# xyloid/a_dive_into_ray_tracing

Hardware: AMD Instinct MI355X
Metric: Msamples/sec (pixels x spp) on RTIOW final scene (higher is better)
Workload: dtype f32

## Files before the change

### a_dive_into_ray_tracing_amd/csrc/rtmi_device.hip

```cpp
#include <hip/hip_runtime.h>
#include <hipcub/hipcub.hpp>

#include <algorithm>
#include <cmath>
#include <cstdint>
#include <cstdlib>
#include <cstdio>
#include <cstring>
#include <memory>
#include <mutex>
#include <string>
#include <vector>

#include "rtmi_internal.h"
#include "rtmi_path.h"


namespace rtmi {

struct RenderArgs {
  Cam<float> cam;
  int32_t n, npairs, W, H, spp, max_depth;
  uint64_t seed;
  int32_t row0, row_step, nrows_valid;
  int32_t tiles_x, n_items;
  int32_t tiles, spp1, chunk1, nch1, chunk2, nch2;
  int32_t block_flush;
  int32_t block_owns_tile;
  int32_t acc_off;
  int32_t s_base;
  uint64_t out_elems;
  Accel acc;
  const int32_t *tile_order;
  unsigned *tile_cost;
};

#ifndef RTMI_WAVES_PER_BLOCK
#define RTMI_WAVES_PER_BLOCK 4
#endif
constexpr int kWavesPerBlock = RTMI_WAVES_PER_BLOCK;
#ifndef RTMI_WAVES_PER_EU
#define RTMI_WAVES_PER_EU 1
#endif
#ifndef RTMI_TRACE
#define RTMI_TRACE 0
#endif
#if RTMI_TRACE
constexpr unsigned kTraceCap = 1u << 18;
__device__ unsigned long long g_trace[kTraceCap * 4];
// ... 121 lines not shown
  atomicAdd(&segments[2], (unsigned long long)cnt.bvh_stats[3]);
  atomicAdd(&segments[4], (unsigned long long)cnt.bvh_stats[4]);
#else
  (void)cnt, (void)lane, (void)segments;
#endif
}

constexpr bool acc_grid(int A) { return A >= 2; }
constexpr bool acc_flat(int A) { return A == 3 || A == 5; }
constexpr bool acc_gmem(int A) { return A >= 4; }

template <int ACC, bool FIRST = false>
__device__ __forceinline__ bool path_segment(const SceneView<float> &sc, const SpherePair *__restrict__ pairs,
                                             const RenderArgs &a, V3<float> &o, V3<float> &d, V3<float> &T,
                                             int &depth, Xoro &rng, V3<float> &col, SegCounters &cnt,
                                             unsigned long long *segments) {
  (void)cnt, (void)segments;
  float t;
#if RTMI_TRACE
  const unsigned long long cyc0 = __builtin_amdgcn_s_memtime();
#endif
  int k;
  uint32_t key = 0u;
  if constexpr (ACC == 1) {
    k = hit_world_bvh<kBigGroup>(a.acc, o, d, t
#if RTMI_STATS
                                  , cnt.bvh_stats
#endif
    );
  } else if constexpr (ACC >= 2) {
    k = hit_world_grid<kBigGroup, acc_flat(ACC), acc_gmem(ACC)>(a.acc, o, d, t, key
#if RTMI_STATS
                                   , cnt.bvh_stats
#endif
#if RTMI_TRACE_PHASES
                                   , cnt.pc
#endif
                                   );
  } else {
    k = hit_world_packed<kPairGroup>(pairs, a.npairs, o, d, t
#if RTMI_STATS
                                     , cnt.stats
#endif
    );
  }
#if RTMI_TRACE
  if constexpr (!(RTMI_TRACE_PHASES && acc_grid(ACC))) cnt.cyc_hit += __builtin_amdgcn_s_memtime() - cyc0;
#endif
#if RTMI_CHECK
  if (k >= a.n) atomicAdd(&segments[7], 1ull << 32);
#endif
  const bool miss = k < 0 || (RTMI_CHECK && k >= a.n);
  const int kk = miss ? 0 : k;
// ... 73 lines not shown
      const int i2 = it - a.tiles * a.nch1;
      tl = i2 / a.nch2;
      sb = a.spp1 + (i2 - tl * a.nch2) * a.chunk2;
      n = max(0, min(a.chunk2, a.spp - sb));
    }
  };
  int tile, s0, ns;
  item_range(has_item ? item : 0, tile, s0, ns);
  if (!has_item) ns = 0;
  if (a.tile_order) tile = a.tile_order[tile];
  const int ty = tile / a.tiles_x, tx = tile - ty * a.tiles_x;
  const int x0 = tx * TW, y0 = ty * TH;
  const int vw = min(TW, a.W - x0), vh = min(TH, a.nrows_valid - y0);
  const int nv = vw * vh;
  const int nq = nv * ns;

  unsigned nseg = 0;
  RTMI_TRACE_BEGIN
  SegCounters cnt{};
#if RTMI_TRACE_PHASES
  unsigned long long cyc_iter = 0, cyc_regen = 0, cyc_ramp = 0;
#endif

  const SceneView<float> sc{geom, sh0, sh1, a.n};

  V3<float> o, d, T;
  int pxd = 0;
  bool active = true;
  Xoro rng;

// ... 44 lines not shown
      unsigned below = 0;
      asm volatile("" : "+s"(below));
      return int(__builtin_amdgcn_mbcnt_hi(~0u, __builtin_amdgcn_mbcnt_lo(~0u, below)));
    };
    const int q = pbase + lane_now();
    const int nvalid = min(64, nq - pbase);
    if constexpr (BATCH) {
#if RTMI_TRACE_PHASES
      const unsigned long long cyc_r = __builtin_amdgcn_s_memtime();
#endif
      bool survives = false;
      if (q < nq) {
        camera_ray(q, po, pd, prng);
        V3<float> unused_T = mk(1.f, 1.f, 1.f), col = mk(0.f, 0.f, 0.f);
        int hit = 0;
        survives = !path_segment<ACC, true>(sc, pairs, a, po, pd, unused_T, hit, prng, col, cnt, segments);
        const int px = job_pixel(pbase + lane_now());
        ptag = px | (hit << 6);
        if (!survives) {
          atomicAdd(&acc[px], (unsigned long long)to_fixed(col.x));
          atomicAdd(&acc[64 + px], (unsigned long long)to_fixed(col.y));
          atomicAdd(&acc[128 + px], (unsigned long long)to_fixed(col.z));
        }
      }
      nseg = unsigned(__builtin_amdgcn_readfirstlane(int(nseg + unsigned(nvalid))));
      const unsigned long long m = __ballot(survives);
      plive = __popcll(m);
      const int rank = __builtin_amdgcn_mbcnt_hi(unsigned(m >> 32), __builtin_amdgcn_mbcnt_lo(unsigned(m), 0u));
      const int dst4 = (survives ? rank : plive + lane_now() - rank) << 2;
      po = mk(push(dst4, po.x), push(dst4, po.y), push(dst4, po.z));
      pd = mk(push(dst4, pd.x), push(dst4, pd.y), push(dst4, pd.z));
// ... 709 lines not shown
  BvhNode *nodes = nullptr;
  int32_t nnodes = 0;
  bool bvh_global = false;
  bool force_bvh_global = std::getenv("RTMI_BVH_GLOBAL") && std::atoi(std::getenv("RTMI_BVH_GLOBAL")) != 0;
  float4 *bvh_sph = nullptr;
  int32_t *bvh_idx = nullptr;
  int32_t nbvh_sph = 0;
  float4 *grid_sph = nullptr;
  uint32_t *grid_cells = nullptr;
  uint32_t *grid_refs = nullptr;
  GridDesc grid{};
  int32_t ngrid_sph = 0;
  bool grid_ok = false;
  bool grid_global = false;
  char *grid_gmem = nullptr;
  bool force_grid_global = std::getenv("RTMI_GRID_GLOBAL") && std::atoi(std::getenv("RTMI_GRID_GLOBAL")) != 0;
  int32_t ordering = RT_ORDER_COST;
  bool block_flush = !(std::getenv("RTMI_BLOCK_FLUSH") && std::getenv("RTMI_BLOCK_FLUSH")[0] == '0');
  bool block_owns = !(std::getenv("RTMI_BLOCK_OWNS") && std::getenv("RTMI_BLOCK_OWNS")[0] == '0');
  int32_t last_sched[8] = {0, 0, 0, 0, 0, 0, 0, 0};
  unsigned *cost_prev = nullptr, *cost_cur = nullptr, *cost_sorted = nullptr;
  int32_t *order = nullptr, *iota = nullptr;
  size_t cost_cap = 0;
  void *sort_tmp = nullptr;
  size_t sort_tmp_bytes = 0;
  bool cost_valid = false;
  int64_t cost_key[6] = {0, 0, 0, 0, 0, 0};
  hipStream_t last_stream = nullptr;
  hipEvent_t last_done = nullptr;
  int32_t tile_w = 0;
// ... 96 lines not shown
    ctx->cu_count = prop.multiProcessorCount;
  }
  *out = ctx.release();
  return RT_OK;
}

RTMI_EXPORT int rt_ctx_destroy(rt_ctx *ctx) {
  if (!ctx) return RT_OK;
  DeviceGuard guard(ctx->device);
  (void)hipStreamSynchronize(ctx->stream);
  for (void *p : {(void *)ctx->geom, (void *)ctx->sh0, (void *)ctx->sh1, (void *)ctx->geom64, (void *)ctx->sh064,
                  (void *)ctx->sh164, (void *)ctx->accum, (void *)ctx->scratch, (void *)ctx->segments, (void *)ctx->pairs, (void *)ctx->counter, (void *)ctx->pass_accum,
                  (void *)ctx->big_pairs, (void *)ctx->big_idx, (void *)ctx->nodes, (void *)ctx->bvh_sph, (void *)ctx->bvh_idx,
                  (void *)ctx->cost_prev, (void *)ctx->cost_cur, (void *)ctx->cost_sorted, (void *)ctx->order,
                  (void *)ctx->iota, ctx->sort_tmp, (void *)ctx->grid_sph, (void *)ctx->grid_cells, (void *)ctx->grid_refs,
                  (void *)ctx->grid_gmem})
    if (p) (void)hipFree(p);
  (void)hipStreamDestroy(ctx->stream);
  if (ctx->last_done) (void)hipEventDestroy(ctx->last_done);
  delete ctx;
  return RT_OK;
}

namespace {
constexpr size_t kBvhLdsMax = 64 * 1024;

uint16_t half_bits(_Float16 h) { return __builtin_bit_cast(uint16_t, h); }
uint16_t half_down(double v) {
  _Float16 h = _Float16(v);
  while (double(h) > v) {
    uint16_t b = half_bits(h);
// ... 80 lines not shown
      build(ids + best_mid, cnt - best_mid);
      nd.link = int32_t(nodes.size());
    }
    nodes[me] = nd;
  }
};
}

namespace {
struct GridBuild {
  GridDesc desc{};
  std::vector<float4> sph;
  std::vector<uint32_t> cells;
  std::vector<uint32_t> refs;
  bool fits_lds = true;
};
bool build_grid(const BvhBuilder &b, const std::vector<int32_t> &small, int32_t n, int32_t nbig_slots,
                GridBuild &out) {
  if (n > 65535) return false;
  const char *env = std::getenv("RTMI_GRID_CELLS");
  const double per_sphere = env && std::atof(env) > 0 ? std::atof(env) : 0.3;
  double lo[3] = {INFINITY, INFINITY, INFINITY}, hi[3] = {-INFINITY, -INFINITY, -INFINITY};
  for (int32_t k : small) {
    const double *c = b.cr + 4 * k, R = std::fabs(c[3]) + b.margin(k);
    for (int a = 0; a < 3; ++a) {
      lo[a] = std::min(lo[a], c[a] - R);
      hi[a] = std::max(hi[a], c[a] + R);
    }
  }
  double e[3], vol = 1;
// ... 36 lines not shown
      for (int y = c0[1]; y <= c1[1]; ++y)
        for (int x = c0[0]; x <= c1[0]; ++x)
          lists[size_t(x + out.desc.n[0] * (y + out.desc.n[1] * z))].push_back(uint16_t(k));
  }
  out.sph.assign(b.g.begin(), b.g.begin() + n);
  out.cells.resize(size_t(total) + 1);
  for (int64_t cidx = 0; cidx < total; ++cidx) {
    out.cells[size_t(cidx)] = uint32_t(out.refs.size());
    for (uint16_t k : lists[size_t(cidx)]) out.refs.push_back(uint32_t(k) * 16u);
  }
  out.cells[size_t(total)] = uint32_t(out.refs.size());
  out.desc.nrefs = int32_t(out.refs.size());
  out.desc.cells_off = 16u * uint32_t(nbig_slots + out.desc.nrefs);
  out.desc.idx_off = out.desc.cells_off + 4u * uint32_t(out.desc.ncells + 1);
  const char *lim_env = std::getenv("RTMI_GRID_LDS_MAX");
  const size_t lds_max = lim_env && std::atoll(lim_env) > 0 ? size_t(std::atoll(lim_env)) : 160 * 1024 / 8 - 3 * 64 * 8 - 256;
  out.fits_lds = grid_lds_bytes(nbig_slots, out.desc.ncells, out.desc.nrefs) <= lds_max;
  return true;
}
}

RTMI_EXPORT int rt_ctx_set_ordering(rt_ctx *ctx, int32_t ordering) {
  if (!ctx) return set_error(RT_EINVAL, "null ctx");
  if (ordering != RT_ORDER_NONE && ordering != RT_ORDER_COST) return set_error(RT_EINVAL, "unknown ordering %d", ordering);
  ctx->ordering = ordering;
  ctx->cost_valid = false;
  return RT_OK;
}

RTMI_EXPORT int rt_ctx_set_accel(rt_ctx *ctx, int32_t accel) {
  if (!ctx) return set_error(RT_EINVAL, "null ctx");
  if (accel != RT_ACCEL_NONE && accel != RT_ACCEL_BVH && accel != RT_ACCEL_GRID)
    return set_error(RT_EINVAL, "unknown accel %d", accel);
// ... 115 lines not shown
    ctx->grid_ok = false;
    GridBuild gb;
    if (!small.empty() && build_grid(b, small, n, nb_pad, gb)) {
      if ((rc = dev_alloc(&ctx->grid_sph, gb.sph.size())) || (rc = dev_alloc(&ctx->grid_cells, gb.cells.size())) ||
          (rc = dev_alloc(&ctx->grid_refs, std::max<size_t>(gb.refs.size(), 1))))
        return rc;
      HIP_TRY(hipMemcpy(ctx->grid_sph, gb.sph.data(), gb.sph.size() * sizeof(float4), hipMemcpyHostToDevice));
      HIP_TRY(hipMemcpy(ctx->grid_cells, gb.cells.data(), gb.cells.size() * sizeof(uint32_t), hipMemcpyHostToDevice));
      if (!gb.refs.empty())
        HIP_TRY(hipMemcpy(ctx->grid_refs, gb.refs.data(), gb.refs.size() * sizeof(uint32_t), hipMemcpyHostToDevice));
      ctx->grid = gb.desc;
      ctx->grid.cells = ctx->grid_cells;
      ctx->grid.refs = ctx->grid_refs;
      ctx->ngrid_sph = int32_t(gb.sph.size());
      ctx->grid_global = ctx->force_grid_global || !gb.fits_lds;
      if (ctx->grid_global) {
        const int32_t nbs = nb_pad, nrec = nbs + gb.desc.nrefs;
        std::vector<char> img(grid_lds_bytes(nbs, gb.desc.ncells, gb.desc.nrefs), 0);
        float4 *rec = reinterpret_cast<float4 *>(img.data());
        uint32_t *cst = reinterpret_cast<uint32_t *>(img.data() + gb.desc.cells_off);
        uint16_t *ix = reinterpret_cast<uint16_t *>(img.data() + gb.desc.idx_off);
        for (int32_t i = 0; i < nrec; ++i) {
          const int32_t k = i < nbs ? bidx[size_t(i)] : int32_t(gb.refs[size_t(i - nbs)] >> 4);
          rec[i] = k < 0 ? make_float4(0.f, 0.f, 0.f, 0.f) : gb.sph[size_t(k)];
          ix[i] = uint16_t(k < 0 ? 0 : k);
        }
        for (int32_t i = 0; i <= gb.desc.ncells; ++i) cst[i] = 16u * (uint32_t(nbs) + gb.cells[size_t(i)]);
        if ((rc = dev_alloc(&ctx->grid_gmem, img.size()))) return rc;
        HIP_TRY(hipMemcpy(ctx->grid_gmem, img.data(), img.size(), hipMemcpyHostToDevice));
      }
// ... 11 lines not shown
  if (n_refs) *n_refs = ctx->grid.nrefs;
  if (lds_bytes) *lds_bytes = int32_t(grid_lds_bytes(2 * ctx->nbig_pairs, ctx->grid.ncells, ctx->grid.nrefs));
  return RT_OK;
}

RTMI_EXPORT int rt_debug_grid_strides(const int32_t *n3, uint32_t *strides2) {
  if (!n3 || !strides2) return set_error(RT_EINVAL, "rt_debug_grid_strides: bad argument");
  GridDesc d{};
  for (int a = 0; a < 3; ++a) d.n[a] = n3[a];
  if (!grid_strides(d)) return set_error(RT_EINVAL, "grid of %d x %d x %d cells: over the walk's 24-bit bound", n3[0], n3[1], n3[2]);
  strides2[0] = d.row_bytes;
  strides2[1] = d.layer_bytes;
  return RT_OK;
}

RTMI_EXPORT int rt_debug_grid_layout(const rt_scene *scene, int32_t *dims3, uint32_t *strides2, float *box6) {
  if (!scene || scene->n <= 0 || !scene->center_radius || !dims3 || !strides2)
    return set_error(RT_EINVAL, "rt_debug_grid_layout: bad argument");
  const int n = scene->n;
  std::vector<float4> g(n, make_float4(0.f, 0.f, 0.f, 0.f));
  std::vector<double> rad(n);
  for (int k = 0; k < n; k++) rad[k] = std::fabs(scene->center_radius[4 * k + 3]);
  std::vector<double> sorted_r = rad;
  std::nth_element(sorted_r.begin(), sorted_r.begin() + n / 2, sorted_r.end());
  const double med = sorted_r[n / 2];
  std::vector<int32_t> big, small;
  double scale = 0;
  for (int k = 0; k < n; k++) {
    (rad[k] > RTMI_BIG_FACTOR * med ? big : small).push_back(k);
    for (int a = 0; a < 3; ++a) scale = std::max(scale, std::fabs(scene->center_radius[4 * k + a]) + rad[k]);
  }
  BvhBuilder b{scene->center_radius, g, 1e-6 * scale, {}, {}, {}};
  const int nb_pad = big.empty() ? 0 : (int(big.size()) + 2 * kBigGroup - 1) / (2 * kBigGroup) * (2 * kBigGroup);
  GridBuild gb;
  if (small.empty() || !build_grid(b, small, n, nb_pad, gb)) return set_error(RT_EUNSUPPORTED, "no grid for this scene");
  for (int a = 0; a < 3; ++a) dims3[a] = gb.desc.n[a];
  strides2[0] = gb.desc.row_bytes;
  strides2[1] = gb.desc.layer_bytes;
  if (box6)
    for (int a = 0; a < 3; ++a) {
      box6[a] = gb.desc.g0[a];
      box6[3 + a] = gb.desc.h[a];
    }
  return RT_OK;
}

RTMI_EXPORT int rt_ctx_set_schedule(rt_ctx *ctx, int32_t chunk, int32_t tail_spp, int32_t tail_chunk) {
  if (!ctx) return set_error(RT_EINVAL, "null ctx");
  if (chunk < 0 || tail_chunk < 0) return set_error(RT_EINVAL, "chunk sizes must be >= 0");
  ctx->chunk = chunk;
// ... 12 lines not shown
RTMI_EXPORT int rt_ctx_set_kernel(rt_ctx *ctx, int32_t kind) {
  if (!ctx) return set_error(RT_EINVAL, "null ctx");
  if (kind != RT_KERNEL_GRID && kind != RT_KERNEL_PERSISTENT && kind != RT_KERNEL_AUTO && kind != RT_KERNEL_QUEUE &&
      kind != RT_KERNEL_RESIDENT)
    return set_error(RT_EINVAL, "unknown kernel kind");
  ctx->kernel = kind;
  return RT_OK;
}

static int auto_tile_w(int32_t W, int32_t rows) {
  auto idle = [&](int64_t tw) {
    const int64_t th = 64 / tw;
    return ((W + tw - 1) / tw) * tw * ((rows + th - 1) / th) * th - int64_t(W) * rows;
  };
  return idle(16) < idle(8) ? 16 : 8;
}

RTMI_EXPORT int rt_ctx_set_tuning(rt_ctx *ctx, int32_t tile_w, int32_t chunk) {
  if (!ctx) return set_error(RT_EINVAL, "null ctx");
  if (tile_w != 0 && tile_w != 8 && tile_w != 16 && tile_w != 32 && tile_w != 64)
    return set_error(RT_EINVAL, "tile_w must be 0 (automatic), 8, 16, 32 or 64");
  if (chunk < 0) return set_error(RT_EINVAL, "chunk must be >= 0");
  ctx->tile_w = tile_w;
  ctx->chunk = chunk;
  return RT_OK;
}

namespace {

size_t accel_lds_bytes(const Accel &acc, int kind) {
// ... 5 lines not shown

Accel accel_of(const rt_ctx *ctx, int kind) {
  Accel a{ctx->big_pairs, ctx->big_idx, ctx->nbig_pairs, 0, nullptr, nullptr, nullptr, 0, GridDesc{}};
  if (kind == 1) {
    a.nnodes = ctx->nnodes;
    a.nodes = ctx->nodes;
    a.sph = ctx->bvh_sph;
    a.sph_idx = ctx->bvh_idx;
    a.nsph = ctx->nbvh_sph;
    a.bvh_global = ctx->bvh_global;
  } else if (kind >= 2) {
    a.sph = ctx->grid_sph;
    a.nsph = ctx->ngrid_sph;
    a.grid = ctx->grid;
    a.grid_gmem = ctx->grid_global ? ctx->grid_gmem : nullptr;
  }
  return a;
}

template <int TW>
void launch_persistent(bool chunked, dim3 grid, hipStream_t st, const rt_ctx *ctx, const RenderArgs &a,
                       unsigned long long *accum, float *out) {
  if (chunked)
    hipLaunchKernelGGL((render_persistent<TW, true>), grid, dim3(64 * kWavesPerBlock), 0, st, ctx->geom, ctx->sh0,
                       ctx->sh1, ctx->pairs, a, accum, out, ctx->segments, ctx->counter);
  else
    hipLaunchKernelGGL((render_persistent<TW, false>), grid, dim3(64 * kWavesPerBlock), 0, st, ctx->geom, ctx->sh0,
                       ctx->sh1, ctx->pairs, a, accum, out, ctx->segments, ctx->counter);
}

template <int TW, int ACC>
void launch_tw(bool chunked, dim3 grid, hipStream_t st, const rt_ctx *ctx, const RenderArgs &a,
               unsigned long long *accum, float *out) {
  RenderArgs b = a;
  b.acc_off = int32_t((accel_lds_bytes(a.acc, ACC) + 15) / 16 * 16);
  const size_t lds = size_t(b.acc_off) + size_t(chunked && a.block_flush ? 1 : GridShape<ACC != 0>::waves) * 3 * 64 * 8;
  if (chunked)
    hipLaunchKernelGGL((render_kernel<TW, true, ACC>), grid, dim3(64 * GridShape<ACC != 0>::waves), lds, st, ctx->geom,
                       ctx->sh0, ctx->sh1, ctx->pairs, b, accum, out, ctx->segments);
  else
    hipLaunchKernelGGL((render_kernel<TW, false, ACC>), grid, dim3(64 * GridShape<ACC != 0>::waves), lds, st, ctx->geom,
                       ctx->sh0, ctx->sh1, ctx->pairs, b, accum, out, ctx->segments);
}

#if RTMI_EXPERIMENTAL
int res_resident_blocks(rt_ctx *ctx, size_t dyn) {
  if (ctx->res_blocks <= 0 || ctx->res_lds != dyn) {
    int per_cu = 0;
    if (hipOccupancyMaxActiveBlocksPerMultiprocessor(&per_cu, (const void *)render_resident<8, 3>, 64 * kResWaves,
                                                     dyn) != hipSuccess)
      per_cu = 0;
// ... 112 lines not shown
  a.npairs = ctx->npairs;
  a.W = W; a.H = H; a.spp = spp; a.max_depth = max_depth; a.seed = seed;
  a.row0 = row0; a.row_step = row_step; a.nrows_valid = nvalid;
  a.tiles_x = tiles_x; a.n_items = int32_t(items);
  a.tiles = int32_t(tiles); a.spp1 = spp1; a.chunk1 = chunk1; a.nch1 = nch1; a.chunk2 = chunk2; a.nch2 = nch2;
  a.block_flush = !persistent && !resident && nch1 % grid_wpb == 0 && nch2 % grid_wpb == 0 && ctx->block_flush;
  a.block_owns_tile = a.block_flush && !pass_accum && nch1 == grid_wpb && nch2 == 0 && ctx->block_owns;
  if (resident) a.block_owns_tile = !pass_accum && nch1 == 1 && nch2 == 0 && ctx->block_owns;
  const bool chunked = pass_accum || nch1 + nch2 > 1;
  if (!ctx->probing) {
    const int32_t sched[8] = {TW, chunk1, nch1, nch2, a.block_flush + a.block_owns_tile, persistent ? 0 : 1,
                              resident ? 3 : (persistent ? 1 : 0), acc_kind == 3 ? 2 : (acc_kind == 5 ? 4 : acc_kind)};
    std::copy(sched, sched + 8, ctx->last_sched);
  }
  a.s_base = s_base;
  a.out_elems = uint64_t(nvalid) * uint64_t(W) * 3;
  const size_t n_valid_out = size_t(nvalid) * W * 3;
  if (chunked && !pass_accum && !a.block_owns_tile) {
    if (ctx->accum_cap < n_valid_out) {
      int rc = dev_alloc(&ctx->accum, n_valid_out);
      if (rc) { ctx->accum_cap = 0; return rc; }
      ctx->accum_cap = n_valid_out;
    }
  }
  unsigned long long *const accum = pass_accum ? pass_accum : ctx->accum;
  if (chunked && !a.block_owns_tile && (!accum || (pass_accum ? ctx->pass_cap : ctx->accum_cap) < n_valid_out))
    return set_error(RT_EHIP, "internal: accumulator not allocated for %zu elements", n_valid_out);
  if ((!chunked || a.block_owns_tile) && !strip) return set_error(RT_EHIP, "internal: no output strip");
  if (int64_t(tiles_y) * TH < nvalid || int64_t(tiles_x) * TW < W || nch1 * int64_t(chunk1) < spp1 ||
      nch2 * int64_t(chunk2) < spp - spp1)
// ... 483 lines not shown
```

### a_dive_into_ray_tracing_amd/csrc/rtmi_path.h

```cpp
#pragma once

#include <hip/hip_runtime.h>

#include <cmath>
#include <cstdint>
#include <type_traits>

#include "../../include/rtmi.h"

#ifndef RTMI_STATS
#define RTMI_STATS 0
#endif

namespace rtmi {


constexpr int kGeomPad = 16;

template <class R> struct V3 { R x, y, z; };
template <class R> __host__ __device__ __forceinline__ V3<R> mk(R x, R y, R z) { return V3<R>{x, y, z}; }

template <bool F> __device__ __forceinline__ float madd(float a, float b, float c) {
  if constexpr (F) return __builtin_fmaf(a, b, c);
  else return a * b + c;
// ... 337 lines not shown
  return true;
}

struct Accel {
  const SpherePair *big;
  const int32_t *big_idx;
  int32_t nbig_pairs;
  int32_t nnodes;
  const BvhNode *nodes;
  const float4 *sph;
  const int32_t *sph_idx;
  int32_t nsph;
  GridDesc grid;
  int32_t bvh_global;
  const char *grid_gmem;
};

__device__ __forceinline__ int32_t big_index(const Accel &a, int slot) {
  typedef const __attribute__((address_space(4))) int32_t *cidx_t;
  return ((cidx_t)(size_t)a.big_idx)[slot];
}

extern __shared__ float4 rtmi_bvh_lds[];
__host__ __device__ constexpr size_t bvh_lds_bytes(int32_t nnodes, int32_t nsph) {
  return size_t(nnodes + nsph) * 16 + size_t(nsph) * 2;
}

__device__ __forceinline__ void stage_bvh(const Accel &g) {
  if (!g.bvh_global) {
    const float4 *nodes = reinterpret_cast<const float4 *>(g.nodes);
    for (int i = threadIdx.x; i < g.nnodes; i += blockDim.x) rtmi_bvh_lds[i] = nodes[i];
// ... 164 lines not shown
      auto res = [&](int slot, float hb, float disc) {
        if constexpr (KEYS)
          resolve_root(int32_t((GMEM ? 0u : lds_address(rtmi_bvh_lds)) + 16u * uint32_t(slot)), hb, disc, inv_a, t_max,
                       best);
        else
          resolve_root(big_index(acc_s, slot), hb, disc, inv_a, t_max, best);
      };
      if (m & 1u) res(2 * q, hb0.x, d0.x);
      if (m & 2u) res(2 * q + 1, hb0.y, d0.y);
      if (m & 4u) res(2 * q + 2, hb1.x, d1.x);
      if (m & 8u) res(2 * q + 3, hb1.y, d1.y);
    }
  }
}

template <int GP, bool FLAT_Y = false, bool GMEM = false>
__device__ __forceinline__ int32_t hit_world_grid(const Accel &acc_s, V3<float> o, V3<float> d, float &t_hit,
                                                  uint32_t &hit_key
#if RTMI_STATS
                                                  , unsigned *gstats
#endif
#if RTMI_TRACE_PHASES
                                                  , PhaseClock &pc
#endif
                                                  ) {
#if RTMI_TRACE_PHASES
  const unsigned long long tp0 = __builtin_amdgcn_s_memtime();
#endif
  RTMI_RAY_TERMS(o, d)
  const char *const gm = GMEM ? acc_s.grid_gmem : nullptr;
  const uint32_t base = GMEM ? 0u : lds_address(rtmi_bvh_lds), idx_base = base + acc_s.grid.idx_off;
  auto rd_u32 = [&](uint32_t addr) {
    if constexpr (GMEM) return *reinterpret_cast<const uint32_t *>(gm + addr);
    else return lds_u32(addr);
  };
  auto rd_u16 = [&](uint32_t addr) {
    if constexpr (GMEM) return uint32_t(*reinterpret_cast<const uint16_t *>(gm + addr));
    else return lds_u16(addr);
  };
  auto rd_sphere = [&](uint32_t addr) {
    if constexpr (GMEM) return *reinterpret_cast<const float4 *>(gm + addr);
    else return lds_sphere(addr);
  };
  float t_max = INFINITY;
  int32_t best_a = -1;
  hit_big<GP, true, GMEM>(acc_s, d, K, a, aL, mx, my, mz, inv_a, t_max, best_a
#if RTMI_STATS
              , gstats
#endif
              );
#if RTMI_TRACE_PHASES
  const unsigned long long tp1 = __builtin_amdgcn_s_memtime();
  pc.c[0] += tp1 - tp0;
  unsigned long long tp2 = tp1;
#endif
  const GridDesc &G = rtmi_grid_desc;
  const float ix = safe_inv<FLAT_Y>(d.x), iy = safe_inv<FLAT_Y>(d.y), iz = safe_inv<FLAT_Y>(d.z);
  const float ox = -o.x * ix, oy = -o.y * iy, oz = -o.z * iz;
  const float bx0 = __builtin_fmaf(G.g0[0], ix, ox), bx1 = __builtin_fmaf(G.g1[0], ix, ox);
  const float by0 = __builtin_fmaf(G.g0[1], iy, oy), by1 = __builtin_fmaf(G.g1[1], iy, oy);
  const float bz0 = __builtin_fmaf(G.g0[2], iz, oz), bz1 = __builtin_fmaf(G.g1[2], iz, oz);
  const float tnear = __builtin_fmaxf(__builtin_fmaxf(__builtin_fminf(bx0, bx1), __builtin_fminf(by0, by1)),
                                      __builtin_fmaxf(__builtin_fminf(bz0, bz1), 0.0f));
  const float tfar = __builtin_fminf(__builtin_fminf(__builtin_fmaxf(bx0, bx1), __builtin_fmaxf(by0, by1)),
                                     __builtin_fminf(__builtin_fmaxf(bz0, bz1), t_max));
  if (tnear <= tfar) {
    const uint32_t cells = base + G.cells_off;
    auto cell_of = [&](float p, int ax) {
      return __builtin_amdgcn_fmed3f(__builtin_floorf((p - G.g0[ax]) * G.inv_h[ax]), 0.0f, G.nm1[ax]);
    };
    const float fx = cell_of(__builtin_fmaf(tnear, d.x, o.x), 0);
    const float fy = FLAT_Y ? 0.0f : cell_of(__builtin_fmaf(tnear, d.y, o.y), 1);
    const float fz = cell_of(__builtin_fmaf(tnear, d.z, o.z), 2);
    const int cx = int(fx), cy = int(fy), cz = int(fz);
    float t0x, t0y, t0z, dtx, dty, dtz, kmx, kmy, kmz;
    auto axis = [&](float inv, float oo, float cf, int ax, float &t0, float &dt, float &kmax) {
      const bool pos = inv >= 0.0f;
      t0 = __builtin_fmaf(__builtin_fmaf(pos ? cf + 1.0f : cf, G.h[ax], G.g0[ax]), inv, oo);
      dt = __builtin_fabsf(G.h[ax] * inv);
      kmax = pos ? G.nm1[ax] - cf : cf;
    };
    axis(ix, ox, fx, 0, t0x, dtx, kmx);
    if constexpr (FLAT_Y) {
      t0y = __builtin_fmaf(__builtin_fmaf(iy >= 0.0f ? 1.0f : 0.0f, G.h[1], G.g0[1]), iy, oy);
      dty = kmy = 0.0f;
    } else {
      axis(iy, oy, fy, 1, t0y, dty, kmy);
    }
    axis(iz, oz, fz, 2, t0z, dtz, kmz);
    float kx = 0.0f, ky = 0.0f, kz = 0.0f, tnx = t0x, tny = t0y, tnz = t0z;
    uint32_t cell = cells + 4u * uint32_t(cx) + __umul24(uint32_t(cz), G.layer_bytes);
    if constexpr (!FLAT_Y) cell += __umul24(uint32_t(cy), G.row_bytes);
    const int dcx = ix >= 0.0f ? 4 : -4;
    const int dcy = FLAT_Y ? 0 : (iy >= 0.0f ? int(G.row_bytes) : -int(G.row_bytes));
    const int dcz = iz >= 0.0f ? int(G.layer_bytes) : -int(G.layer_bytes);
#if RTMI_TRACE_PHASES
    tp2 = __builtin_amdgcn_s_memtime();
#endif
    for (;;) {
#if RTMI_STATS
      gstats[0] += 1;
      if (__lane_id() == __builtin_ctzll(__ballot(1))) gstats[2] += 1;
#endif
      const uint32_t re = rd_u32(cell + 4u);
      constexpr uint32_t kNoKey = 0xFFFFFFFFu;
      uint32_t kaddr = kNoKey;
      float khb = 0.0f, kdisc = 0.0f;
      for (uint32_t r = rd_u32(cell); r < re; r += 16u) {
#if RTMI_STATS
        gstats[1] += 1;
        if (__lane_id() == __builtin_ctzll(__ballot(1))) gstats[3] += 1;
#endif
        float hb, disc;
        sphere_test(rd_sphere(r), d, K, a, aL, mx, my, mz, hb, disc);
        if (!(disc < 0.0f)) {
          if (kaddr != kNoKey) {
#if RTMI_STATS
            if (__lane_id() == __builtin_ctzll(__ballot(1))) gstats[4] += 1;
#endif
            resolve_key<GMEM>(kaddr, khb, kdisc, inv_a, t_max, best_a, idx_base, gm);
          }
          kaddr = r;
          khb = hb;
          kdisc = disc;
        }
      }
      if (kaddr != kNoKey) {
#if RTMI_STATS
        if (__lane_id() == __builtin_ctzll(__ballot(1))) gstats[4] += 1;
#endif
        resolve_key<GMEM>(kaddr, khb, kdisc, inv_a, t_max, best_a, idx_base, gm);
      }
      const float texit = __builtin_fminf(tnx, __builtin_fminf(tny, tnz));
      if constexpr (FLAT_Y) {
        const bool sx = (tnx <= tny) & (tnx <= tnz);
        const bool sy = !sx & (tny <= tnz);
        const bool leave = !(texit < t_max) | sy | ((sx ? kx : kz) >= (sx ? kmx : kmz));
        if (leave) break;
        kx = sx ? kx + 1.0f : kx;
        kz = sx ? kz : kz + 1.0f;
        tnx = sx ? __builtin_fmaf(kx, dtx, t0x) : tnx;
        tnz = sx ? tnz : __builtin_fmaf(kz, dtz, t0z);
        cell += sx ? dcx : dcz;
        continue;
      }
      if (!(texit < t_max)) break;
      if (tnx <= tny && tnx <= tnz) {
        if (kx >= kmx) break;
        kx += 1.0f;
        tnx = __builtin_fmaf(kx, dtx, t0x);
        cell += dcx;
      } else if (tny <= tnz) {
        if (FLAT_Y || ky >= kmy) break;
        ky += 1.0f;
        tny = __builtin_fmaf(ky, dty, t0y);
        cell += dcy;
      } else {
        if (kz >= kmz) break;
        kz += 1.0f;
        tnz = __builtin_fmaf(kz, dtz, t0z);
        cell += dcz;
      }
    }
  }
#if RTMI_TRACE_PHASES
  {
    const unsigned long long tp3 = __builtin_amdgcn_s_memtime();
    pc.c[1] += tp2 - tp1;
    pc.c[2] += tp3 - tp2;
  }
#endif
  t_hit = t_max;
  hit_key = best_a < 0 ? base : uint32_t(best_a);
  const int32_t k = int32_t(rd_u16(idx_base + ((hit_key - base) >> 3)));
  return best_a < 0 ? -1 : k;
}
// ... 191 lines not shown
```

Measured before the change: 27710.

## Add per-tile camera-ray candidate sphere lists to skip grid traversal

Before tracing a tile, each wave builds a conservative list of small spheres that any primary ray from that tile's pixel cone could hit, and stores their LDS record keys in a per-wave LDS region. First-bounce grid hits then test only those candidates instead of walking the grid cells. The list is used only when it fits the cap and the tile has enough samples. This adds a per-tile culling pass over all small spheres, extra LDS, and a smaller grid LDS budget. For tiles with many candidates it falls back to normal traversal.

```diff
diff --git a/a_dive_into_ray_tracing_amd/csrc/rtmi_device.hip b/a_dive_into_ray_tracing_amd/csrc/rtmi_device.hip
--- a/a_dive_into_ray_tracing_amd/csrc/rtmi_device.hip
+++ b/a_dive_into_ray_tracing_amd/csrc/rtmi_device.hip
@@ -33,6 +33,7 @@
   Accel acc;
   const int32_t *tile_order;
   unsigned *tile_cost;
+  int32_t tile_list_max;
 };
 
 #ifndef RTMI_WAVES_PER_BLOCK
@@ -184,8 +185,8 @@
 __device__ __forceinline__ bool path_segment(const SceneView<float> &sc, const SpherePair *__restrict__ pairs,
                                              const RenderArgs &a, V3<float> &o, V3<float> &d, V3<float> &T,
                                              int &depth, Xoro &rng, V3<float> &col, SegCounters &cnt,
-                                             unsigned long long *segments) {
-  (void)cnt, (void)segments;
+                                             unsigned long long *segments, int32_t tile_list = -1) {
+  (void)cnt, (void)segments, (void)tile_list;
   float t;
 #if RTMI_TRACE
   const unsigned long long cyc0 = __builtin_amdgcn_s_memtime();
@@ -199,14 +200,14 @@
 #endif
     );
   } else if constexpr (ACC >= 2) {
-    k = hit_world_grid<kBigGroup, acc_flat(ACC), acc_gmem(ACC)>(a.acc, o, d, t, key
+    k = hit_world_grid<kBigGroup, acc_flat(ACC), acc_gmem(ACC), FIRST && !acc_gmem(ACC)>(a.acc, o, d, t, key
 #if RTMI_STATS
                                    , cnt.bvh_stats
 #endif
 #if RTMI_TRACE_PHASES
                                    , cnt.pc
 #endif
-                                   );
+                                   , tile_list);
   } else {
     k = hit_world_packed<kPairGroup>(pairs, a.npairs, o, d, t
 #if RTMI_STATS
@@ -310,6 +311,35 @@
   const int vw = min(TW, a.W - x0), vh = min(TH, a.nrows_valid - y0);
   const int nv = vw * vh;
   const int nq = nv * ns;
+
+  int32_t tile_list = -1;
+  if constexpr (ACC == 2 || ACC == 3) {
+    uint16_t *const tl = reinterpret_cast<uint16_t *>(acc_lds + (acc_shared ? 1 : WPB) * 3 * 64) + wave * kTileListCap;
+    const int cap = min(a.tile_list_max, kTileListCap);
+    if (cap > 0 && ns >= kTileListMinSpp && a.acc.ntile > 0) {
+      const TileBundle tb = tile_bundle(a.cam, a.W, a.H, x0, vw, a.row0 + y0 * a.row_step,
+                                        a.row0 + (y0 + vh - 1) * a.row_step);
+      const uint32_t *const keys = reinterpret_cast<const uint32_t *>(a.acc.tile_sph + a.acc.ntile);
+      const int ln = int(__builtin_amdgcn_mbcnt_hi(~0u, __builtin_amdgcn_mbcnt_lo(~0u, 0u)));
+      int n = 0;
+      for (int i0 = 0; i0 < a.acc.ntile && n <= cap; i0 += 64) {
+        const int i = i0 + ln;
+        bool pass = false;
+        uint32_t key = 0u;
+        if (i < a.acc.ntile) {
+          const float4 s = a.acc.tile_sph[i];
+          key = keys[i];
+          pass = tile_may_hit(tb, s.x, s.y, s.z, s.w);
+        }
+        const unsigned long long m = __ballot(pass);
+        const int slot = n + int(__builtin_amdgcn_mbcnt_hi(unsigned(m >> 32), __builtin_amdgcn_mbcnt_lo(unsigned(m), 0u)));
+        if (pass && slot < cap) tl[slot] = uint16_t(key);
+        n = __builtin_amdgcn_readfirstlane(n + __popcll(m));
+      }
+      __builtin_amdgcn_fence(__ATOMIC_RELEASE, "wavefront");
+      if (n <= cap) tile_list = __builtin_amdgcn_readfirstlane(int(lds_address(tl) << 6) | n);
+    }
+  }
 
   unsigned nseg = 0;
   RTMI_TRACE_BEGIN
@@ -384,7 +414,7 @@
         camera_ray(q, po, pd, prng);
         V3<float> unused_T = mk(1.f, 1.f, 1.f), col = mk(0.f, 0.f, 0.f);
         int hit = 0;
-        survives = !path_segment<ACC, true>(sc, pairs, a, po, pd, unused_T, hit, prng, col, cnt, segments);
+        survives = !path_segment<ACC, true>(sc, pairs, a, po, pd, unused_T, hit, prng, col, cnt, segments, tile_list);
         const int px = job_pixel(pbase + lane_now());
         ptag = px | (hit << 6);
         if (!survives) {
@@ -1124,6 +1154,11 @@
   bool grid_ok = false;
   bool grid_global = false;
   char *grid_gmem = nullptr;
+  float4 *tile_sph = nullptr;
+  int32_t ntile = 0;
+  int32_t tile_list_max = std::getenv("RTMI_TILE_LIST_MAX")
+                              ? std::max(0, std::min(kTileListCap, std::atoi(std::getenv("RTMI_TILE_LIST_MAX"))))
+                              : kTileListCap;
   bool force_grid_global = std::getenv("RTMI_GRID_GLOBAL") && std::atoi(std::getenv("RTMI_GRID_GLOBAL")) != 0;
   int32_t ordering = RT_ORDER_COST;
   bool block_flush = !(std::getenv("RTMI_BLOCK_FLUSH") && std::getenv("RTMI_BLOCK_FLUSH")[0] == '0');
@@ -1250,7 +1285,7 @@
                   (void *)ctx->big_pairs, (void *)ctx->big_idx, (void *)ctx->nodes, (void *)ctx->bvh_sph, (void *)ctx->bvh_idx,
                   (void *)ctx->cost_prev, (void *)ctx->cost_cur, (void *)ctx->cost_sorted, (void *)ctx->order,
                   (void *)ctx->iota, ctx->sort_tmp, (void *)ctx->grid_sph, (void *)ctx->grid_cells, (void *)ctx->grid_refs,
-                  (void *)ctx->grid_gmem})
+                  (void *)ctx->grid_gmem, (void *)ctx->tile_sph})
     if (p) (void)hipFree(p);
   (void)hipStreamDestroy(ctx->stream);
   if (ctx->last_done) (void)hipEventDestroy(ctx->last_done);
@@ -1361,6 +1396,8 @@
   std::vector<uint32_t> cells;
   std::vector<uint32_t> refs;
   bool fits_lds = true;
+  std::vector<float4> tile_sph;
+  std::vector<uint32_t> tile_keys;
 };
 bool build_grid(const BvhBuilder &b, const std::vector<int32_t> &small, int32_t n, int32_t nbig_slots,
                 GridBuild &out) {
@@ -1427,9 +1464,32 @@
   out.desc.cells_off = 16u * uint32_t(nbig_slots + out.desc.nrefs);
   out.desc.idx_off = out.desc.cells_off + 4u * uint32_t(out.desc.ncells + 1);
   const char *lim_env = std::getenv("RTMI_GRID_LDS_MAX");
-  const size_t lds_max = lim_env && std::atoll(lim_env) > 0 ? size_t(std::atoll(lim_env)) : 160 * 1024 / 8 - 3 * 64 * 8 - 256;
+  const size_t lds_max = lim_env && std::atoll(lim_env) > 0
+                             ? size_t(std::atoll(lim_env))
+                             : 160 * 1024 / 8 - 3 * 64 * 8 - 256 - GridShape<true>::waves * 2 * kTileListCap;
   out.fits_lds = grid_lds_bytes(nbig_slots, out.desc.ncells, out.desc.nrefs) <= lds_max;
+  std::vector<uint32_t> first(size_t(n), UINT32_MAX);
+  for (size_t p = out.refs.size(); p-- > 0;) first[out.refs[p] >> 4] = uint32_t(nbig_slots) + uint32_t(p);
+  if (size_t(nbig_slots) + out.refs.size() <= 65536) {
+    for (int32_t k : small) {
+      const double *c = b.cr + 4 * k, R = std::fabs(c[3]) + b.margin(k);
+      float rg = float(R);
+      if (double(rg) < R) rg = std::nextafter(rg, INFINITY);
+      out.tile_sph.push_back(make_float4(float(c[0]), float(c[1]), float(c[2]), rg));
+      out.tile_keys.push_back(first[size_t(k)]);
+    }
+  }
   return true;
+}
+
+void tile_extent(int32_t W, int32_t row0, int32_t row_step, int32_t nvalid, int32_t tw, int32_t tile, int32_t &x0,
+                 int32_t &vw, int32_t &j_lo, int32_t &j_hi) {
+  const int32_t th = 64 / tw, tiles_x = (W + tw - 1) / tw, ty = tile / tiles_x, tx = tile - ty * tiles_x;
+  const int32_t y0 = ty * th, vh = std::min(th, nvalid - y0);
+  x0 = tx * tw;
+  vw = std::min(tw, W - x0);
+  j_lo = row0 + y0 * row_step;
+  j_hi = row0 + (y0 + vh - 1) * row_step;
 }
 }
 
@@ -1575,6 +1635,16 @@
       ctx->grid.refs = ctx->grid_refs;
       ctx->ngrid_sph = int32_t(gb.sph.size());
       ctx->grid_global = ctx->force_grid_global || !gb.fits_lds;
+      ctx->ntile = 0;
+      if (!ctx->grid_global && !gb.tile_sph.empty()) {
+        const size_t ns = gb.tile_sph.size();
+        std::vector<float4> tab(ns + (ns + 3) / 4);
+        std::copy(gb.tile_sph.begin(), gb.tile_sph.end(), tab.begin());
+        std::memcpy(tab.data() + ns, gb.tile_keys.data(), ns * sizeof(uint32_t));
+        if ((rc = dev_alloc(&ctx->tile_sph, tab.size()))) return rc;
+        HIP_TRY(hipMemcpy(ctx->tile_sph, tab.data(), tab.size() * sizeof(float4), hipMemcpyHostToDevice));
+        ctx->ntile = int32_t(ns);
+      }
       if (ctx->grid_global) {
         const int32_t nbs = nb_pad, nrec = nbs + gb.desc.nrefs;
         std::vector<char> img(grid_lds_bytes(nbs, gb.desc.ncells, gb.desc.nrefs), 0);
@@ -1616,9 +1686,8 @@
   return RT_OK;
 }
 
-RTMI_EXPORT int rt_debug_grid_layout(const rt_scene *scene, int32_t *dims3, uint32_t *strides2, float *box6) {
-  if (!scene || scene->n <= 0 || !scene->center_radius || !dims3 || !strides2)
-    return set_error(RT_EINVAL, "rt_debug_grid_layout: bad argument");
+namespace {
+bool host_grid(const rt_scene *scene, GridBuild &gb, int32_t &nbs) {
   const int n = scene->n;
   std::vector<float4> g(n, make_float4(0.f, 0.f, 0.f, 0.f));
   std::vector<double> rad(n);
@@ -1633,9 +1702,17 @@
     for (int a = 0; a < 3; ++a) scale = std::max(scale, std::fabs(scene->center_radius[4 * k + a]) + rad[k]);
   }
   BvhBuilder b{scene->center_radius, g, 1e-6 * scale, {}, {}, {}};
-  const int nb_pad = big.empty() ? 0 : (int(big.size()) + 2 * kBigGroup - 1) / (2 * kBigGroup) * (2 * kBigGroup);
+  nbs = big.empty() ? 0 : (int(big.size()) + 2 * kBigGroup - 1) / (2 * kBigGroup) * (2 * kBigGroup);
+  return !small.empty() && build_grid(b, small, n, nbs, gb);
+}
+}
+
+RTMI_EXPORT int rt_debug_grid_layout(const rt_scene *scene, int32_t *dims3, uint32_t *strides2, float *box6) {
+  if (!scene || scene->n <= 0 || !scene->center_radius || !dims3 || !strides2)
+    return set_error(RT_EINVAL, "rt_debug_grid_layout: bad argument");
   GridBuild gb;
-  if (small.empty() || !build_grid(b, small, n, nb_pad, gb)) return set_error(RT_EUNSUPPORTED, "no grid for this scene");
+  int32_t nb_pad;
+  if (!host_grid(scene, gb, nb_pad)) return set_error(RT_EUNSUPPORTED, "no grid for this scene");
   for (int a = 0; a < 3; ++a) dims3[a] = gb.desc.n[a];
   strides2[0] = gb.desc.row_bytes;
   strides2[1] = gb.desc.layer_bytes;
@@ -1678,6 +1755,37 @@
     return ((W + tw - 1) / tw) * tw * ((rows + th - 1) / th) * th - int64_t(W) * rows;
   };
   return idle(16) < idle(8) ? 16 : 8;
+}
+
+RTMI_EXPORT int rt_debug_tile_list(const rt_scene *scene, const rt_camera *camera, int32_t W, int32_t H, int32_t row0,
+                                   int32_t row_step, int32_t nrows, int32_t tile_w, int32_t tile, int32_t cap,
+                                   int32_t *out_indices, int32_t *out_count) {
+  if (!scene || scene->n <= 0 || !scene->center_radius || !camera || !out_indices || !out_count)
+    return set_error(RT_EINVAL, "rt_debug_tile_list: bad argument");
+  if (W < 2 || H < 2 || row0 < 0 || row0 >= H || row_step < 1 || nrows < 1 || cap < 1 || cap > kTileListCap ||
+      (tile_w != 0 && tile_w != 8 && tile_w != 16 && tile_w != 32 && tile_w != 64))
+    return set_error(RT_EINVAL, "rt_debug_tile_list: bad image, strip, tile shape or cap");
+  const int32_t nvalid = int32_t(std::min<int64_t>(nrows, (int64_t(H) - row0 + row_step - 1) / row_step));
+  const int32_t tw = tile_w ? tile_w : auto_tile_w(W, nvalid), th = 64 / tw;
+  const int64_t tiles = int64_t((W + tw - 1) / tw) * ((nvalid + th - 1) / th);
+  if (tile < -1 || tile >= tiles) return set_error(RT_EINVAL, "rt_debug_tile_list: tile %d of %lld", tile, (long long)tiles);
+  GridBuild gb;
+  int32_t nbs;
+  if (!host_grid(scene, gb, nbs) || gb.tile_sph.empty()) return set_error(RT_EUNSUPPORTED, "no tile lists for this scene");
+  const Cam<float> cam = cam_f(camera);
+  for (int64_t t = tile < 0 ? 0 : tile, o = 0; t < (tile < 0 ? tiles : tile + 1); ++t, ++o) {
+    int32_t x0, vw, j_lo, j_hi, cnt = 0;
+    tile_extent(W, row0, row_step, nvalid, tw, int32_t(t), x0, vw, j_lo, j_hi);
+    const TileBundle tb = tile_bundle(cam, W, H, x0, vw, j_lo, j_hi);
+    for (size_t i = 0; i < gb.tile_sph.size(); ++i) {
+      const float4 s = gb.tile_sph[i];
+      if (!tile_may_hit(tb, s.x, s.y, s.z, s.w)) continue;
+      if (cnt < cap) out_indices[o * cap + cnt] = int32_t(gb.refs[gb.tile_keys[i] - uint32_t(nbs)] >> 4);
+      ++cnt;
+    }
+    out_count[o] = cnt <= cap ? cnt : -1;
+  }
+  return RT_OK;
 }
 
 RTMI_EXPORT int rt_ctx_set_tuning(rt_ctx *ctx, int32_t tile_w, int32_t chunk) {
@@ -1713,6 +1821,8 @@
     a.nsph = ctx->ngrid_sph;
     a.grid = ctx->grid;
     a.grid_gmem = ctx->grid_global ? ctx->grid_gmem : nullptr;
+    a.tile_sph = ctx->tile_sph;
+    a.ntile = kind <= 3 ? ctx->ntile : 0;
   }
   return a;
 }
@@ -1733,7 +1843,8 @@
                unsigned long long *accum, float *out) {
   RenderArgs b = a;
   b.acc_off = int32_t((accel_lds_bytes(a.acc, ACC) + 15) / 16 * 16);
-  const size_t lds = size_t(b.acc_off) + size_t(chunked && a.block_flush ? 1 : GridShape<ACC != 0>::waves) * 3 * 64 * 8;
+  const size_t lds = size_t(b.acc_off) + size_t(chunked && a.block_flush ? 1 : GridShape<ACC != 0>::waves) * 3 * 64 * 8 +
+                     (ACC == 2 || ACC == 3 ? size_t(GridShape<true>::waves) * 2 * kTileListCap : 0);
   if (chunked)
     hipLaunchKernelGGL((render_kernel<TW, true, ACC>), grid, dim3(64 * GridShape<ACC != 0>::waves), lds, st, ctx->geom,
                        ctx->sh0, ctx->sh1, ctx->pairs, b, accum, out, ctx->segments);
@@ -1876,6 +1987,7 @@
     std::copy(sched, sched + 8, ctx->last_sched);
   }
   a.s_base = s_base;
+  a.tile_list_max = ctx->tile_list_max;
   a.out_elems = uint64_t(nvalid) * uint64_t(W) * 3;
   const size_t n_valid_out = size_t(nvalid) * W * 3;
   if (chunked && !pass_accum && !a.block_owns_tile) {
diff --git a/a_dive_into_ray_tracing_amd/csrc/rtmi_path.h b/a_dive_into_ray_tracing_amd/csrc/rtmi_path.h
--- a/a_dive_into_ray_tracing_amd/csrc/rtmi_path.h
+++ b/a_dive_into_ray_tracing_amd/csrc/rtmi_path.h
@@ -375,7 +375,56 @@
   GridDesc grid;
   int32_t bvh_global;
   const char *grid_gmem;
+  const float4 *tile_sph;
+  int32_t ntile;
 };
+
+struct TileBundle {
+  float ox, oy, oz;
+  float ex, ey, ez;
+  float rho;
+  float k;
+  float q;
+};
+constexpr int kTileListCap = 32;
+constexpr int kTileListMinSpp = 4;
+
+__host__ __device__ inline TileBundle tile_bundle(const Cam<float> &c, int32_t W, int32_t H, int32_t x0, int32_t vw,
+                                                  int32_t j_lo, int32_t j_hi) {
+  const float s0 = float(x0) / float(W - 1), s1 = float(x0 + vw) / float(W - 1);
+  const float t0 = float(j_lo) / float(H - 1), t1 = float(j_hi + 1) / float(H - 1);
+  const float sc = 0.5f * (s0 + s1), tc = 0.5f * (t0 + t1), sh = 0.5f * (s1 - s0), th = 0.5f * (t1 - t0);
+  const float dx = c.llc.x + sc * c.hor.x + tc * c.ver.x - c.origin.x;
+  const float dy = c.llc.y + sc * c.hor.y + tc * c.ver.y - c.origin.y;
+  const float dz = c.llc.z + sc * c.hor.z + tc * c.ver.z - c.origin.z;
+  const float ax = sh * c.hor.x, ay = sh * c.hor.y, az = sh * c.hor.z;
+  const float bx = th * c.ver.x, by = th * c.ver.y, bz = th * c.ver.z;
+  const float aa = ax * ax + ay * ay + az * az, bb = bx * bx + by * by + bz * bz, ab = ax * bx + ay * by + az * bz;
+  const float rf = sqrtf(aa + bb + 2.0f * fabsf(ab));
+  const float uu = c.u.x * c.u.x + c.u.y * c.u.y + c.u.z * c.u.z, vv = c.v.x * c.v.x + c.v.y * c.v.y + c.v.z * c.v.z;
+  const float uv = c.u.x * c.v.x + c.u.y * c.v.y + c.u.z * c.v.z;
+  const float hd = 0.5f * (uu - vv);
+  const float rho = fabsf(c.lens) * sqrtf(0.5f * (uu + vv) + sqrtf(hd * hd + uv * uv));
+  const float len = sqrtf(dx * dx + dy * dy + dz * dz), inv = 1.0f / len;
+  TileBundle b;
+  b.ox = c.origin.x; b.oy = c.origin.y; b.oz = c.origin.z;
+  b.ex = dx * inv; b.ey = dy * inv; b.ez = dz * inv;
+  const float on = fmaxf(fmaxf(fabsf(c.origin.x), fabsf(c.origin.y)), fabsf(c.origin.z));
+  b.rho = 1.001f * rho + 1e-5f * (1.0f + on);
+  b.k = 1.001f * ((rf + rho) * inv) + 1e-5f;
+  b.q = fmaxf(0.0f, 1.0f - b.k * b.k);
+  return b;
+}
+
+__host__ __device__ inline bool tile_may_hit(const TileBundle &b, float cx, float cy, float cz, float rg) {
+  const float px = cx - b.ox, py = cy - b.oy, pz = cz - b.oz;
+  const float al = px * b.ex + py * b.ey + pz * b.ez;
+  const float tau = fmaxf(al, 0.0f);
+  const float qx = px - tau * b.ex, qy = py - tau * b.ey, qz = pz - tau * b.ez;
+  const float h2 = qx * qx + qy * qy + qz * qz;
+  const float rhs = rg + b.rho + b.k * tau;
+  return !(h2 * b.q > rhs * rhs);
+}
 
 __device__ __forceinline__ int32_t big_index(const Accel &a, int slot) {
   typedef const __attribute__((address_space(4))) int32_t *cidx_t;
@@ -570,7 +619,7 @@
   }
 }
 
-template <int GP, bool FLAT_Y = false, bool GMEM = false>
+template <int GP, bool FLAT_Y = false, bool GMEM = false, bool LIST = false>
 __device__ __forceinline__ int32_t hit_world_grid(const Accel &acc_s, V3<float> o, V3<float> d, float &t_hit,
                                                   uint32_t &hit_key
 #if RTMI_STATS
@@ -579,7 +628,8 @@
 #if RTMI_TRACE_PHASES
                                                   , PhaseClock &pc
 #endif
-                                                  ) {
+                                                  , int32_t tile_list = -1) {
+  static_assert(!(LIST && GMEM), "tile lists name LDS record slots");
 #if RTMI_TRACE_PHASES
   const unsigned long long tp0 = __builtin_amdgcn_s_memtime();
 #endif
@@ -610,112 +660,131 @@
   pc.c[0] += tp1 - tp0;
   unsigned long long tp2 = tp1;
 #endif
-  const GridDesc &G = rtmi_grid_desc;
-  const float ix = safe_inv<FLAT_Y>(d.x), iy = safe_inv<FLAT_Y>(d.y), iz = safe_inv<FLAT_Y>(d.z);
-  const float ox = -o.x * ix, oy = -o.y * iy, oz = -o.z * iz;
-  const float bx0 = __builtin_fmaf(G.g0[0], ix, ox), bx1 = __builtin_fmaf(G.g1[0], ix, ox);
-  const float by0 = __builtin_fmaf(G.g0[1], iy, oy), by1 = __builtin_fmaf(G.g1[1], iy, oy);
-  const float bz0 = __builtin_fmaf(G.g0[2], iz, oz), bz1 = __builtin_fmaf(G.g1[2], iz, oz);
-  const float tnear = __builtin_fmaxf(__builtin_fmaxf(__builtin_fminf(bx0, bx1), __builtin_fminf(by0, by1)),
-                                      __builtin_fmaxf(__builtin_fminf(bz0, bz1), 0.0f));
-  const float tfar = __builtin_fminf(__builtin_fminf(__builtin_fmaxf(bx0, bx1), __builtin_fmaxf(by0, by1)),
-                                     __builtin_fminf(__builtin_fmaxf(bz0, bz1), t_max));
-  if (tnear <= tfar) {
-    const uint32_t cells = base + G.cells_off;
-    auto cell_of = [&](float p, int ax) {
-      return __builtin_amdgcn_fmed3f(__builtin_floorf((p - G.g0[ax]) * G.inv_h[ax]), 0.0f, G.nm1[ax]);
-    };
-    const float fx = cell_of(__builtin_fmaf(tnear, d.x, o.x), 0);
-    const float fy = FLAT_Y ? 0.0f : cell_of(__builtin_fmaf(tnear, d.y, o.y), 1);
-    const float fz = cell_of(__builtin_fmaf(tnear, d.z, o.z), 2);
-    const int cx = int(fx), cy = int(fy), cz = int(fz);
-    float t0x, t0y, t0z, dtx, dty, dtz, kmx, kmy, kmz;
-    auto axis = [&](float inv, float oo, float cf, int ax, float &t0, float &dt, float &kmax) {
-      const bool pos = inv >= 0.0f;
-      t0 = __builtin_fmaf(__builtin_fmaf(pos ? cf + 1.0f : cf, G.h[ax], G.g0[ax]), inv, oo);
-      dt = __builtin_fabsf(G.h[ax] * inv);
-      kmax = pos ? G.nm1[ax] - cf : cf;
-    };
-    axis(ix, ox, fx, 0, t0x, dtx, kmx);
-    if constexpr (FLAT_Y) {
-      t0y = __builtin_fmaf(__builtin_fmaf(iy >= 0.0f ? 1.0f : 0.0f, G.h[1], G.g0[1]), iy, oy);
-      dty = kmy = 0.0f;
-    } else {
-      axis(iy, oy, fy, 1, t0y, dty, kmy);
+  if (LIST && tile_list >= 0) {
+    const uint32_t tl = uint32_t(tile_list) >> 6, tl_end = tl + 2u * (uint32_t(tile_list) & 63u);
+    for (uint32_t e = tl; e < tl_end; e += 2u) {
+      const uint32_t key = base + 16u * uint32_t(__builtin_amdgcn_readfirstlane(int(lds_u16(e))));
+#if RTMI_STATS
+      gstats[1] += 1;
+      if (__lane_id() == __builtin_ctzll(__ballot(1))) gstats[3] += 1;
+#endif
+      float hb, disc;
+      sphere_test(rd_sphere(key), d, K, a, aL, mx, my, mz, hb, disc);
+      if (!(disc < 0.0f)) {
+#if RTMI_STATS
+        if (__lane_id() == __builtin_ctzll(__ballot(1))) gstats[4] += 1;
+#endif
+        resolve_key<GMEM>(key, hb, disc, inv_a, t_max, best_a, idx_base, gm);
+      }
     }
-    axis(iz, oz, fz, 2, t0z, dtz, kmz);
-    float kx = 0.0f, ky = 0.0f, kz = 0.0f, tnx = t0x, tny = t0y, tnz = t0z;
-    uint32_t cell = cells + 4u * uint32_t(cx) + __umul24(uint32_t(cz), G.layer_bytes);
-    if constexpr (!FLAT_Y) cell += __umul24(uint32_t(cy), G.row_bytes);
-    const int dcx = ix >= 0.0f ? 4 : -4;
-    const int dcy = FLAT_Y ? 0 : (iy >= 0.0f ? int(G.row_bytes) : -int(G.row_bytes));
-    const int dcz = iz >= 0.0f ? int(G.layer_bytes) : -int(G.layer_bytes);
+  } else {
+    const GridDesc &G = rtmi_grid_desc;
+    const float ix = safe_inv<FLAT_Y>(d.x), iy = safe_inv<FLAT_Y>(d.y), iz = safe_inv<FLAT_Y>(d.z);
+    const float ox = -o.x * ix, oy = -o.y * iy, oz = -o.z * iz;
+    const float bx0 = __builtin_fmaf(G.g0[0], ix, ox), bx1 = __builtin_fmaf(G.g1[0], ix, ox);
+    const float by0 = __builtin_fmaf(G.g0[1], iy, oy), by1 = __builtin_fmaf(G.g1[1], iy, oy);
+    const float bz0 = __builtin_fmaf(G.g0[2], iz, oz), bz1 = __builtin_fmaf(G.g1[2], iz, oz);
+    const float tnear = __builtin_fmaxf(__builtin_fmaxf(__builtin_fminf(bx0, bx1), __builtin_fminf(by0, by1)),
+                                        __builtin_fmaxf(__builtin_fminf(bz0, bz1), 0.0f));
+    const float tfar = __builtin_fminf(__builtin_fminf(__builtin_fmaxf(bx0, bx1), __builtin_fmaxf(by0, by1)),
+                                       __builtin_fminf(__builtin_fmaxf(bz0, bz1), t_max));
+    if (tnear <= tfar) {
+      const uint32_t cells = base + G.cells_off;
+      auto cell_of = [&](float p, int ax) {
+        return __builtin_amdgcn_fmed3f(__builtin_floorf((p - G.g0[ax]) * G.inv_h[ax]), 0.0f, G.nm1[ax]);
+      };
+      const float fx = cell_of(__builtin_fmaf(tnear, d.x, o.x), 0);
+      const float fy = FLAT_Y ? 0.0f : cell_of(__builtin_fmaf(tnear, d.y, o.y), 1);
+      const float fz = cell_of(__builtin_fmaf(tnear, d.z, o.z), 2);
+      const int cx = int(fx), cy = int(fy), cz = int(fz);
+      float t0x, t0y, t0z, dtx, dty, dtz, kmx, kmy, kmz;
+      auto axis = [&](float inv, float oo, float cf, int ax, float &t0, float &dt, float &kmax) {
+        const bool pos = inv >= 0.0f;
+        t0 = __builtin_fmaf(__builtin_fmaf(pos ? cf + 1.0f : cf, G.h[ax], G.g0[ax]), inv, oo);
+        dt = __builtin_fabsf(G.h[ax] * inv);
+        kmax = pos ? G.nm1[ax] - cf : cf;
+      };
+      axis(ix, ox, fx, 0, t0x, dtx, kmx);
+      if constexpr (FLAT_Y) {
+        t0y = __builtin_fmaf(__builtin_fmaf(iy >= 0.0f ? 1.0f : 0.0f, G.h[1], G.g0[1]), iy, oy);
+        dty = kmy = 0.0f;
+      } else {
+        axis(iy, oy, fy, 1, t0y, dty, kmy);
+      }
+      axis(iz, oz, fz, 2, t0z, dtz, kmz);
+      float kx = 0.0f, ky = 0.0f, kz = 0.0f, tnx = t0x, tny = t0y, tnz = t0z;
+      uint32_t cell = cells + 4u * uint32_t(cx) + __umul24(uint32_t(cz), G.layer_bytes);
+      if constexpr (!FLAT_Y) cell += __umul24(uint32_t(cy), G.row_bytes);
+      const int dcx = ix >= 0.0f ? 4 : -4;
+      const int dcy = FLAT_Y ? 0 : (iy >= 0.0f ? int(G.row_bytes) : -int(G.row_bytes));
+      const int dcz = iz >= 0.0f ? int(G.layer_bytes) : -int(G.layer_bytes);
 #if RTMI_TRACE_PHASES
-    tp2 = __builtin_amdgcn_s_memtime();
-#endif
-    for (;;) {
-#if RTMI_STATS
-      gstats[0] += 1;
-      if (__lane_id() == __builtin_ctzll(__ballot(1))) gstats[2] += 1;
-#endif
-      const uint32_t re = rd_u32(cell + 4u);
-      constexpr uint32_t kNoKey = 0xFFFFFFFFu;
-      uint32_t kaddr = kNoKey;
-      float khb = 0.0f, kdisc = 0.0f;
-      for (uint32_t r = rd_u32(cell); r < re; r += 16u) {
-#if RTMI_STATS
-        gstats[1] += 1;
-        if (__lane_id() == __builtin_ctzll(__ballot(1))) gstats[3] += 1;
-#endif
-        float hb, disc;
-        sphere_test(rd_sphere(r), d, K, a, aL, mx, my, mz, hb, disc);
-        if (!(disc < 0.0f)) {
-          if (kaddr != kNoKey) {
-#if RTMI_STATS
-            if (__lane_id() == __builtin_ctzll(__ballot(1))) gstats[4] += 1;
-#endif
-            resolve_key<GMEM>(kaddr, khb, kdisc, inv_a, t_max, best_a, idx_base, gm);
+      tp2 = __builtin_amdgcn_s_memtime();
+#endif
+      for (;;) {
+#if RTMI_STATS
+        gstats[0] += 1;
+        if (__lane_id() == __builtin_ctzll(__ballot(1))) gstats[2] += 1;
+#endif
+        const uint32_t re = rd_u32(cell + 4u);
+        constexpr uint32_t kNoKey = 0xFFFFFFFFu;
+        uint32_t kaddr = kNoKey;
+        float khb = 0.0f, kdisc = 0.0f;
+        for (uint32_t r = rd_u32(cell); r < re; r += 16u) {
+#if RTMI_STATS
+          gstats[1] += 1;
+          if (__lane_id() == __builtin_ctzll(__ballot(1))) gstats[3] += 1;
+#endif
+          float hb, disc;
+          sphere_test(rd_sphere(r), d, K, a, aL, mx, my, mz, hb, disc);
+          if (!(disc < 0.0f)) {
+            if (kaddr != kNoKey) {
+#if RTMI_STATS
+              if (__lane_id() == __builtin_ctzll(__ballot(1))) gstats[4] += 1;
+#endif
+              resolve_key<GMEM>(kaddr, khb, kdisc, inv_a, t_max, best_a, idx_base, gm);
+            }
+            kaddr = r;
+            khb = hb;
+            kdisc = disc;
           }
-          kaddr = r;
-          khb = hb;
-          kdisc = disc;
         }
-      }
-      if (kaddr != kNoKey) {
-#if RTMI_STATS
-        if (__lane_id() == __builtin_ctzll(__ballot(1))) gstats[4] += 1;
-#endif
-        resolve_key<GMEM>(kaddr, khb, kdisc, inv_a, t_max, best_a, idx_base, gm);
-      }
-      const float texit = __builtin_fminf(tnx, __builtin_fminf(tny, tnz));
-      if constexpr (FLAT_Y) {
-        const bool sx = (tnx <= tny) & (tnx <= tnz);
-        const bool sy = !sx & (tny <= tnz);
-        const bool leave = !(texit < t_max) | sy | ((sx ? kx : kz) >= (sx ? kmx : kmz));
-        if (leave) break;
-        kx = sx ? kx + 1.0f : kx;
-        kz = sx ? kz : kz + 1.0f;
-        tnx = sx ? __builtin_fmaf(kx, dtx, t0x) : tnx;
-        tnz = sx ? tnz : __builtin_fmaf(kz, dtz, t0z);
-        cell += sx ? dcx : dcz;
-        continue;
-      }
-      if (!(texit < t_max)) break;
-      if (tnx <= tny && tnx <= tnz) {
-        if (kx >= kmx) break;
-        kx += 1.0f;
-        tnx = __builtin_fmaf(kx, dtx, t0x);
-        cell += dcx;
-      } else if (tny <= tnz) {
-        if (FLAT_Y || ky >= kmy) break;
-        ky += 1.0f;
-        tny = __builtin_fmaf(ky, dty, t0y);
-        cell += dcy;
-      } else {
-        if (kz >= kmz) break;
-        kz += 1.0f;
-        tnz = __builtin_fmaf(kz, dtz, t0z);
-        cell += dcz;
+        if (kaddr != kNoKey) {
+#if RTMI_STATS
+          if (__lane_id() == __builtin_ctzll(__ballot(1))) gstats[4] += 1;
+#endif
+          resolve_key<GMEM>(kaddr, khb, kdisc, inv_a, t_max, best_a, idx_base, gm);
+        }
+        const float texit = __builtin_fminf(tnx, __builtin_fminf(tny, tnz));
+        if constexpr (FLAT_Y) {
+          const bool sx = (tnx <= tny) & (tnx <= tnz);
+          const bool sy = !sx & (tny <= tnz);
+          const bool leave = !(texit < t_max) | sy | ((sx ? kx : kz) >= (sx ? kmx : kmz));
+          if (leave) break;
+          kx = sx ? kx + 1.0f : kx;
+          kz = sx ? kz : kz + 1.0f;
+          tnx = sx ? __builtin_fmaf(kx, dtx, t0x) : tnx;
+          tnz = sx ? tnz : __builtin_fmaf(kz, dtz, t0z);
+          cell += sx ? dcx : dcz;
+          continue;
+        }
+        if (!(texit < t_max)) break;
+        if (tnx <= tny && tnx <= tnz) {
+          if (kx >= kmx) break;
+          kx += 1.0f;
+          tnx = __builtin_fmaf(kx, dtx, t0x);
+          cell += dcx;
+        } else if (tny <= tnz) {
+          if (FLAT_Y || ky >= kmy) break;
+          ky += 1.0f;
+          tny = __builtin_fmaf(ky, dty, t0y);
+          cell += dcy;
+        } else {
+          if (kz >= kmz) break;
+          kz += 1.0f;
+          tnz = __builtin_fmaf(kz, dtz, t0z);
+          cell += dcz;
+        }
       }
     }
   }
```

Result: faster. 28970 (median of 6 runs) (+4.5%).
